# mit-acl/rl_collision_avoidance

Measured on AMD Instinct MI355X. Metric: agent-steps/sec (env.step) at 4 agents x 8192 worlds per GPU, higher is better.
Workload: dtype f64

## Files before the change

### __graft_entry__.py

```python
import os
import sys

ROOT = os.path.dirname(os.path.abspath(__file__))
if ROOT not in sys.path:
    sys.path.insert(0, ROOT)


def build() -> None:
    from rl_collision_avoidance_amd import build as hip_build
    path = hip_build.build(verbose=True)
    assert os.path.exists(path)
    try:
        for kind in (1, 2, 3, 4):
            hip_build.build_ulp_fault(kind)
    except Exception as exc:
        print("warning: development variant not built (%s); the tests that need it build it themselves" % exc)
    try:
        hip_build.build_crowd_dev()
    except Exception as exc:
        print("warning: crowd development variant not built (%s); tests/test_gpu_crowd.py builds it itself" % exc)
    from oracle import c_oracle
    c_oracle.build()
    import rl_collision_avoidance_amd
    from rl_collision_avoidance_amd import _lib
    handle = _lib.lib()
    for name, _, _ in _lib.SYMBOLS:
        getattr(handle, name)
    print("build ok:", path)


def smoke() -> None:
    import numpy as np
    import torch
    from oracle import c_oracle as co
    from rl_collision_avoidance_amd.batched_env import BatchedCollisionAvoidanceEnv

    assert torch.cuda.is_available(), "smoke() needs cuda:0"
    W, N, seed = 256, 4, 17
    env = BatchedCollisionAvoidanceEnv(W, device="cuda:0", seed=seed)
    env.reset()
    ocfg, ogen = co.default_cfg(N), co.default_gen(N, N, pool_size=int(env.cfg.gen_pool_size))
    st = co.State.empty(W, N)
    ep = np.zeros(W, np.uint32)
    co.generate(ocfg, ogen, seed, st, ep)
    rng = np.random.default_rng(seed)
    for t in range(40):
        acts = rng.integers(0, 11, size=(W, N)).astype(np.int32)
        obs, rew, done, go = env.step_autoreset(torch.from_numpy(acts).cuda())
        oobs, orew, odone, ogo = co.step_autoreset(ocfg, ogen, seed, st, ep, acts)
        assert np.array_equal(done.cpu().numpy(), odone) and np.array_equal(go.cpu().numpy(), ogo)
        d = np.abs(obs.cpu().numpy() - oobs)
        d[..., 3] = np.minimum(d[..., 3], np.abs(d[..., 3] - 2 * np.pi))
        assert d.max() <= 1e-5
        assert np.abs(rew.cpu().numpy() - orew).max() <= 1e-5
    fl = env.get_state()[2].cpu().numpy().view(np.uint32)
    assert np.array_equal(fl, st.flags)
    acts16 = rng.integers(0, 11, size=(16, W, N)).astype(np.int32)
    slots = env.new_step_slots(16, packed=True)
    pk_all, go_all = env.step_autoreset_packed(torch.from_numpy(acts16).cuda(), slots)
    wdt = env.obs_width
    for k in range(16):
        oobs, orew, odone, ogo = co.step_autoreset(ocfg, ogen, seed, st, ep, acts16[k])
        pk = pk_all[k].cpu().numpy()
        d = np.abs(pk[..., :wdt] - oobs)
        d[..., 3] = np.minimum(d[..., 3], np.abs(d[..., 3] - 2 * np.pi))
        assert d.max() <= 1e-5 and np.abs(pk[..., wdt] - orew).max() <= 1e-5, k
        assert np.array_equal(pk[..., wdt + 1].astype(np.uint8), odone) and np.array_equal(go_all[k].cpu().numpy(), ogo), k
    assert np.array_equal(env.get_state()[2].cpu().numpy().view(np.uint32), st.flags)
    obs = torch.from_numpy(np.ascontiguousarray(pk[..., :wdt])).cuda()
    from rl_collision_avoidance_amd.ga3c.network import NetworkVP_rnn
    from rl_collision_avoidance_amd.ga3c.policy_kernel import FusedPolicy
    net = NetworkVP_rnn(env.config).to("cuda:0")
    view = obs.view(W * N, -1)[:, 1:]
# ... 44 lines not shown
```

### rl_collision_avoidance_amd/build.py

```python
from __future__ import annotations

import os
import shutil
import subprocess

PKG_DIR = os.path.dirname(os.path.abspath(__file__))
ROOT = os.path.dirname(PKG_DIR)
CSRC = os.path.join(PKG_DIR, "csrc")
LIB_PATH = os.path.join(PKG_DIR, "libcavoid_hip.so")
SOURCES = [os.path.join(CSRC, "cavoid_capi.hip"), os.path.join(CSRC, "cavoid_multistep.hip"), os.path.join(CSRC, "cavoid_rvo.hip"),
           os.path.join(CSRC, "cavoid_relay.hip"), os.path.join(CSRC, "cavoid_quad.hip"), os.path.join(CSRC, "cavoid_rollout_capi.hip"),
           os.path.join(CSRC, "cavoid_policy_capi.hip"), os.path.join(CSRC, "cavoid_comm_capi.hip"), os.path.join(CSRC, "cavoid_actor.hip"),
           os.path.join(CSRC, "cavoid_actor_rvo.hip"), os.path.join(CSRC, "cavoid_actor_frozen.hip"), os.path.join(CSRC, "cavoid_crowd.hip"),
           os.path.join(CSRC, "cavoid_policy_ws.hip"), os.path.join(CSRC, "cavoid_policy_train_ring.hip"),
           os.path.join(CSRC, "cavoid_policy_wsring.hip"), os.path.join(CSRC, "cavoid_crowd_push.hip"), os.path.join(CSRC, "cavoid_crowd_rvo.hip"),
           os.path.join(CSRC, "cavoid_crowd_actor.hip")]
HEADERS = {
    "cavoid_capi.hip": ["cavoid_kernels.hpp", "cavoid_launch.hpp", "cavoid_host.hpp", "cavoid_crowd.hpp", "cavoid_crowd_rvo.hpp"],
    "cavoid_multistep.hip": ["cavoid_kernels.hpp", "cavoid_launch.hpp", "cavoid_host.hpp"],
    "cavoid_rvo.hip": ["cavoid_kernels.hpp", "cavoid_launch.hpp", "cavoid_host.hpp"],
    "cavoid_relay.hip": ["cavoid_kernels.hpp", "cavoid_relay.hpp", "cavoid_launch.hpp", "cavoid_host.hpp"],
    "cavoid_quad.hip": ["cavoid_kernels.hpp", "cavoid_quad.hpp", "cavoid_launch.hpp", "cavoid_host.hpp"],
    "cavoid_rollout_capi.hip": ["cavoid_rollout.hpp", "cavoid_rollout_host.hpp", "cavoid_host.hpp"],
    "cavoid_policy_capi.hip": ["cavoid_policy.hpp", "cavoid_policy_split.hpp", "cavoid_policy_split8.hpp", "cavoid_policy_crowd.hpp", "cavoid_policy_host.hpp",
# ... 116 lines not shown
    from concurrent.futures import ThreadPoolExecutor
    out = variant_path("ulp%d" % kind)
    if os.path.exists(out):
        return out
    build()
    objs = _compile_objects([], "", False, verbose)
    jobs, swap = [], {}
    for name in ("cavoid_capi.hip", "cavoid_multistep.hip", "cavoid_rvo.hip", "cavoid_relay.hip"):
        src = os.path.join(CSRC, name)
        obj = os.path.join(OBJ_DIR, name.replace(".hip", ".ulp%d.o" % kind))
        jobs.append([hipcc()] + FLAGS + EXTRA_FLAGS.get(name, []) + ["-DCAVOID_DEV_ULP_FAULT=%d" % kind, "-DCAVOID_DEV_ONLY_N", "-c", src, "-o", obj])
        swap[os.path.join(OBJ_DIR, name.replace(".hip", ".o"))] = obj
    if jobs:
        if verbose:
            for j in jobs:
                print(" ".join(j), flush=True)
        with ThreadPoolExecutor(max_workers=len(jobs)) as pool:
            list(pool.map(subprocess.check_call, jobs))
    for old in glob.glob(os.path.join(FAULT_DIR, "libcavoid_hip_ulp%d-*.so" % kind)):
        os.remove(old)
    tmp = out + ".tmp"
    _link([swap.get(o, o) for o in objs], tmp, verbose)
    os.replace(tmp, out)
    return out


def build_crowd_dev(verbose: bool = False) -> str:
    import glob
    from concurrent.futures import ThreadPoolExecutor
    out = variant_path("crowd2")
    if os.path.exists(out):
        return out
    build()
    objs = _compile_objects([], "", False, verbose)
    jobs, swap = [], {}
    for name in ("cavoid_capi.hip", "cavoid_multistep.hip", "cavoid_crowd.hip", "cavoid_crowd_rvo.hip"):
        src = os.path.join(CSRC, name)
        obj = os.path.join(OBJ_DIR, name.replace(".hip", ".crowd2.o"))
        jobs.append([hipcc()] + FLAGS + EXTRA_FLAGS.get(name, []) + ["-DCAVOID_DEV_CROWD_FROM_N=2", "-DCAVOID_DEV_ONLY_N", "-c", src, "-o", obj])
        swap[os.path.join(OBJ_DIR, name.replace(".hip", ".o"))] = obj
    if verbose:
        for j in jobs:
            print(" ".join(j), flush=True)
    with ThreadPoolExecutor(max_workers=len(jobs)) as pool:
        list(pool.map(subprocess.check_call, jobs))
    for old in glob.glob(os.path.join(FAULT_DIR, "libcavoid_hip_crowd2-*.so")):
        os.remove(old)
    tmp = out + ".tmp"
    _link([swap.get(o, o) for o in objs], tmp, verbose)
    os.replace(tmp, out)
    return out


if __name__ == "__main__":
    import sys
    if "--trace" in sys.argv:
        print(build_trace(verbose=True))
    elif "--crowd-dev" in sys.argv:
        print(build_crowd_dev(verbose=True))
    elif "--ulp-faults" in sys.argv:
        for kind in (1, 2, 3, 4):
            print(build_ulp_fault(kind, verbose=True))
    else:
        print(build(force=True, verbose=True))
```

### rl_collision_avoidance_amd/csrc/cavoid_kernels.hpp

```cpp
#pragma once
#include <hip/hip_runtime.h>
#include <stdint.h>

#include "cavoid.h"

namespace cavoid {

#ifdef CAVOID_TRACE
__device__ unsigned long long *g_trace = nullptr;
#define CAVOID_STAMP(k)                                                                \
    do {                                                                               \
        if (lane == 0 && g_trace) g_trace[wave * 16 + (k)] = (unsigned long long)clock64(); \
    } while (0)
#else
#define CAVOID_STAMP(k) do { } while (0)
#endif

#define CAVOID_RARE(x) __builtin_expect(!!(x), 0)
#ifndef CAVOID_SKIP
#define CAVOID_SKIP 0
#endif

constexpr double kPi = 3.14159265358979323846;
constexpr int kTileMaxAgents = 16;
// ... 255 lines not shown

__device__ __forceinline__ Ego ego_from(const KCfg &c, double tx, double ty, double heading) {
    Ego e;
    e.tx = tx;
    e.ty = ty;
    const double ss = e.tx * e.tx + e.ty * e.ty;
    const bool tiny = !(ss > 1e-16);
    double y = (double)__builtin_amdgcn_rsqf((float)ss);
    y = y * __builtin_fma(-0.5 * ss, y * y, 1.5);
    y = y * __builtin_fma(-0.5 * ss, y * y, 1.5);
    e.dist = tiny ? sqrt(ss) : ss * y;
    const double inv = tiny ? 1.0 : y;
    e.prll_x = e.tx * inv;
    e.prll_y = e.ty * inv;
    e.heading_ego = wrap_once(heading - (double)atan2f((float)e.ty, (float)e.tx), c.switches);
    return e;
}
__device__ __forceinline__ Ego ego_frame_obs(const KCfg &c, const Agent &a) { return ego_from(c, (double)a.gx - a.px, (double)a.gy - a.py, a.heading); }

__device__ __forceinline__ double time_to_impact(double rx, double ry, double vx, double vy, double R) {
    const double cc = rx * rx + ry * ry - R * R;
    if (cc <= 0.0) return 0.0;
    const double aa = vx * vx + vy * vy, bb = rx * vx + ry * vy;
    if (aa < 1e-10 || bb <= 0.0) return INFINITY;
    const double disc = bb * bb - aa * cc;
    if (disc < 0.0) return INFINITY;
    return (bb - sqrt(disc)) / aa;
}

__device__ __forceinline__ double sqrt_dist2(double x) {
    const double y = __builtin_amdgcn_rsq(fmax(x, 0x1p-1000));
    double g = x * y;
    double h = y * 0.5;
    const double r = __builtin_fma(-h, g, 0.5);
    g = __builtin_fma(g, r, g);
    h = __builtin_fma(h, r, h);
    double d = __builtin_fma(-g, g, x);
    g = __builtin_fma(d, h, g);
    d = __builtin_fma(-g, g, x);
    g = __builtin_fma(d, h, g);
    return g;
}

template <int N>
struct Others {
    static constexpr int K = N > 1 ? N - 1 : 1;
};

__device__ __forceinline__ int other_index(int i, int o, int n) {
    const int j = i + 1 + o;
    return j >= n ? j - n : j;
}

__device__ __forceinline__ uint32_t orderable(float f) {
    const uint32_t u = __float_as_uint(f + 0.0f);
    return u ^ ((u >> 31) ? 0xFFFFFFFFu : 0x80000000u);
}

struct Key {
    uint64_t v;
    __device__ __forceinline__ uint32_t hi() const { return (uint32_t)(v >> 32); }
    __device__ __forceinline__ uint32_t lo() const { return (uint32_t)v; }
    __device__ __forceinline__ void set(uint32_t hi, uint32_t lo) { v = ((uint64_t)hi << 32) | lo; }
};
constexpr uint32_t kKeyBias = 1u << 30;
constexpr uint32_t kKeySentinel = 0x7FFFFFF0u;
__device__ __forceinline__ bool key_is_sentinel(uint32_t hi) { return hi >= kKeySentinel; }
__device__ __forceinline__ int key_bucket(const Key &k) { return (int)(kKeyBias - k.hi()); }

struct OtherState { double px, py; float vxf, vyf, r; };

template <int N>
struct RingStage {
    static constexpr bool kDouble = N >= kRingDoubleFromN;
    const StageRec *self;
    const double *vx64, *vy64;
    int i, base;
    __device__ __forceinline__ OtherState other(int o) const {
        const StageRec *q = self + (o + 1);
        if (!kDouble) q = (o + 1 + i >= N) ? q - N : q;
        return OtherState{q->px, q->py, q->vxf, q->vyf, q->r};
    }
    __device__ __forceinline__ void vel64(int o, double &vx, double &vy) const {
        const int j = base + other_index(i, o, N);
        vx = vx64[j]; vy = vy64[j];
    }
};
template <int N>
struct ArrayStage {
    const double *px, *py, *vx, *vy;
    const float *r;
    int i, base;
    __device__ __forceinline__ OtherState other(int o) const {
        const int j = base + other_index(i, o, N);
        return OtherState{px[j], py[j], (float)vx[j], (float)vy[j], r[j]};
    }
    __device__ __forceinline__ void vel64(int o, double &ovx, double &ovy) const {
        const int j = base + other_index(i, o, N);
        ovx = vx[j]; ovy = vy[j];
    }
};

constexpr int kFeat = 5;
__device__ __forceinline__ void neighbour_features(const Ego &e, float pxf, float pyf, double rx, double ry, const OtherState &q, float (&f)[kFeat]) {
    f[0] = (float)__builtin_fma(rx, e.prll_x, ry * e.prll_y);
    f[1] = (float)__builtin_fma(ry, e.prll_x, -(rx * e.prll_y));
#if !defined(CAVOID_DEV_PKFORM)
    float t_par = q.vyf * pyf, t_orth = q.vxf * pyf;
    asm volatile("" : "+v"(t_par), "+v"(t_orth));
    f[2] = __builtin_fmaf(q.vxf, pxf, t_par);
    f[3] = __builtin_fmaf(q.vyf, pxf, -t_orth);
#else
    f[2] = __builtin_fmaf(q.vxf, pxf, q.vyf * pyf);
    f[3] = __builtin_fmaf(q.vyf, pxf, -(q.vxf * pyf));
#endif
    f[4] = q.r;
}

constexpr int kParkFromN = 6;
template <int N, bool PARK, bool SW, bool FEAT, class Stage>
__device__ __forceinline__ void pair_pass_impl(const KCfg &c, const Agent &a, const Ego &e, bool present, const Stage &st,
                                          Key (&key)[Others<N>::K], float (&gapf)[Others<N>::K], float (*feat)[kFeat],
                                          uint32_t &valid, bool &hit, double &min_gap, uint32_t *park, int lane, uint32_t frozen_w) {
    constexpr int K = Others<N>::K;
    const double ri = (double)a.radius;
    valid = 0u;
    hit = false;
    min_gap = INFINITY;
    if (!PARK) { key[0].set(kKeySentinel, 0u); gapf[0] = 0.0f; }
    auto one = [&](int o) {
        const OtherState q = st.other(o);
        const float rjf = q.r;
        const double rx = q.px - a.px, ry = q.py - a.py;
#if defined(CAVOID_DEV_ULP_FAULT) && CAVOID_DEV_ULP_FAULT == 1
        const double d = sqrt_dist2((double)((float)rx * (float)rx) + ry * ry);
#else
        const double d = sqrt_dist2(rx * rx + ry * ry);
#endif
        const bool other = present && (rjf >= 0.0f);
        bool collides = other;
        if (SW) {
            const int jj = other_index(st.i, o, N);
            collides = other && ((frozen_w >> jj) & 1u) == 0u && ((frozen_w >> st.i) & 1u) == 0u;
        }
        const double gap_c = d - (ri + (double)rjf);
        min_gap = collides ? fmin(min_gap, gap_c) : min_gap;
        hit = hit || (collides && gap_c <= c.collision_dist);
        const bool seen = other && !(d > c.horizon);
        valid |= seen ? (1u << o) : 0u;
        const double gap_o = d - ri - (double)rjf;
#if defined(CAVOID_DEV_ULP_FAULT) && CAVOID_DEV_ULP_FAULT == 3
        uint32_t hi = kKeyBias - (uint32_t)(int)rintf((float)gap_o * 100.0f);
#else
        uint32_t hi = kKeyBias - (uint32_t)(int)rint(gap_o * 100.0);
#endif
        uint32_t lo = orderable((float)(ry * e.tx - rx * e.ty));
        if (SW) {
            if (c.switches & kSwIndexTie) lo = (uint32_t)other_index(st.i, o, N);
            if (c.switches & kSwExactGap) { lo = 0u; hi = 0x7FFFFFFEu - (orderable((float)gap_o) >> 1); }
        }
        hi = seen ? hi : kKeySentinel + (uint32_t)o;
        if (PARK) {
            reinterpret_cast<uint64_t *>(park)[o * 64 + lane] = ((uint64_t)hi << 32) | lo;
            park[(2 * K + o) * 64 + lane] = __float_as_uint((float)gap_o);
        } else {
            gapf[o] = (float)gap_o;
            key[o].set(hi, lo);
        }
        if (FEAT) neighbour_features(e, (float)e.prll_x, (float)e.prll_y, rx, ry, q, feat[o]);
    };
    if (PARK) {
#pragma unroll 3
        for (int o = 0; o < N - 1; ++o) { one(o); __builtin_amdgcn_sched_barrier(0); }
    } else {
#pragma unroll
        for (int o = 0; o < N - 1; ++o) if (!(CAVOID_SKIP & 16) || o == 0) one(o);
    }
}

template <int N, bool PARK, bool FEAT, class Stage>
__device__ __forceinline__ void pair_pass(const KCfg &c, const Agent &a, const Ego &e, bool present, const Stage &st,
                                          Key (&key)[Others<N>::K], float (&gapf)[Others<N>::K], float (*feat)[kFeat],
                                          uint32_t &valid, bool &hit, double &min_gap, uint32_t *park = nullptr, int lane = 0,
                                          uint32_t frozen_w = 0u) {
    if (CAVOID_RARE(c.switches != 0u))
        pair_pass_impl<N, PARK, true, FEAT>(c, a, e, present, st, key, gapf, feat, valid, hit, min_gap, park, lane, frozen_w);
    else
        pair_pass_impl<N, PARK, false, FEAT>(c, a, e, present, st, key, gapf, feat, valid, hit, min_gap, park, lane, 0u);
}

#ifndef CAVOID_NT_STORES
// ... 1126 lines not shown
```

### rl_collision_avoidance_amd/csrc/cavoid_launch.hpp

```cpp
#pragma once
#include <hip/hip_runtime.h>
#include <hip/hip_ext.h>

#include <type_traits>

#include "cavoid.h"
#include "cavoid_host.hpp"
#include "cavoid_kernels.hpp"

struct cavoid_env {
    int device = 0;
    int64_t W = 0, A = 0, world_offset = 0;
    cavoid_cfg cfg{};
    cavoid::KCfg k{};
    cavoid::KState st{};
    cavoid::PoolRec *pool = nullptr;
    uint32_t *pool_episode = nullptr;
    int64_t pool_size = 0;
    int ahead_R = 0;
    uint32_t *ahead_hi[2] = {nullptr, nullptr};
    int ahead_cur = 0;
    int ahead_budget = 0;
    bool ahead_primed = false;
    bool ahead_always = false;
    int64_t ahead_refills = 0;
    int relay_topup_nc = -1;
    size_t relay_topup_lds = 0;
    bool relay_topup_fits = false;
    void *slab = nullptr;
    void *pool_slab = nullptr;
    double *d_actions = nullptr;
    int waves_per_block = 4;
    int grid = 0;
    int pipeline = 2;
    int relay_consumers = 3;
    int latency_mode = 0;
    int quad = -1;
    int prefetch_single = 0;
    int last_form = CAVOID_FORM_NONE;
    int last_relay_consumers = 0;
    hipEvent_t ev0 = nullptr, ev1 = nullptr;
};


namespace cavoid {

template <int... Ns>
struct NList {};
#ifdef CAVOID_DEV_ONLY_N
using EnvNs = NList<4, 10>;
using RelayNs = NList<4>;
using QuadNs = NList<4>;
#else
using EnvNs = NList<1, 2, 3, 4, 5, 6, 7, 8, 9, 10, 11, 12, 13, 14, 15, 16>;
using RelayNs = NList<1, 2, 3, 4, 5, 6>;
using QuadNs = NList<2, 3, 4, 5, 6, 10>;
#endif

#ifdef CAVOID_DEV_CROWD_FROM_N
constexpr int kCrowdFromN = CAVOID_DEV_CROWD_FROM_N;
#else
constexpr int kCrowdFromN = kTileMaxAgents + 1;
#endif
static inline bool crowd_form(int max_agents) { return max_agents >= kCrowdFromN; }

template <int... Ns, class F>
static inline int dispatch_n(int n, NList<Ns...>, F &&f) {
    int rc = CAVOID_EUNSUPPORTED;
    (void)((n == Ns ? (rc = f(std::integral_constant<int, Ns>{}), true) : false) || ...);
    return rc;
}

template <class K, class... Args>
static inline void launch_kernel(K kernel, dim3 grid, dim3 block, size_t lds, hipStream_t s, hipEvent_t ev_start, hipEvent_t ev_stop,
                                 const Args &...args) {
    if (ev_start || ev_stop) hipExtLaunchKernelGGL(kernel, grid, block, lds, s, ev_start, ev_stop, 0, args...);
    else hipLaunchKernelGGL(kernel, grid, block, lds, s, args...);
}

#ifdef CAVOID_TRACE
static inline int set_trace(unsigned long long *dev_ptr) {
    HIP_TRY(hipMemcpyToSymbol(HIP_SYMBOL(g_trace), &dev_ptr, sizeof(dev_ptr)));
    return CAVOID_OK;
}
#endif

static inline int note_form(cavoid_env *e, int rc, int form, int relay_consumers = 0) {
    if (rc == CAVOID_OK) {
        e->last_form = form;
        e->last_relay_consumers = relay_consumers;
    }
    return rc;
}

template <int MODE, bool RVO = false>
static inline int launch_on(cavoid_env *e, const KCfg &k, const KState &st, int grid_x, const KIO &io, hipStream_t s,
                     hipEvent_t ev_start, hipEvent_t ev_stop) {
    const dim3 grid(grid_x), block(64 * e->waves_per_block);
    const int row = io.obs ? io.obs_stride : k.width;
    int tile = (k.tile_rows * row + 3) & ~3;
    if (tile < k.park_floats) tile = k.park_floats;
    const size_t lds = (size_t)(lds_floats_block() + e->waves_per_block * (lds_floats_fixed(e->cfg.max_agents) + k.rvo_lds_floats + tile)) * sizeof(float);
    const int rc = dispatch_n(e->cfg.max_agents, EnvNs{}, [&](auto n) -> int {
        launch_kernel(env_kernel<decltype(n)::value, MODE, RVO>, grid, block, lds, s, ev_start, ev_stop, k, st, e->pool, io);
// ... 57 lines not shown
```

### rl_collision_avoidance_amd/csrc/cavoid_relay.hpp

```cpp
#pragma once
#include <cstddef>
#include <type_traits>

#include "cavoid_kernels.hpp"

namespace cavoid {

constexpr int kRelayMaxAgents = 6;
template <int N>
__host__ __device__ constexpr int relay_ring() { return N <= 5 ? 8 : 4; }
constexpr size_t kRelayLdsLimit = 80 * 1024;
constexpr int kRelayActRing = 64;
constexpr int kRelayActAhead = 48;
constexpr int kRelayEvq = 8;
constexpr int kRelayTopupMaxN = 5;

struct RelaySeq {
    int spec;
    int stage;
    int res;
    int fin;
    int act;
    int ev;
    int nxt;
// ... 217 lines not shown
template <int N, bool SW>
__device__ __forceinline__ void relay_pair_part(const KCfg &c, const Agent &a, const Ego &e, const bool present, const ArrayStage<N> &st, const int pw,
                                                const int lane, RelayCoop<N> &co, float (&gapf)[Others<N>::K], float (&feat)[Others<N>::K][kFeat]) {
    const double ri = (double)a.radius;
#pragma unroll
    for (int o = 0; o < N - 1; ++o) {
        if (o % kRelayCoopWaves != pw) continue;
        const OtherState q = st.other(o);
        const float rjf = q.r;
        const double rx = q.px - a.px, ry = q.py - a.py;
#if defined(CAVOID_DEV_ULP_FAULT) && CAVOID_DEV_ULP_FAULT == 1
        const double d = sqrt_dist2((double)((float)rx * (float)rx) + ry * ry);
#else
        const double d = sqrt_dist2(rx * rx + ry * ry);
#endif
        const bool other = present && (rjf >= 0.0f);
        const bool seen = other && !(d > c.horizon);
        const double gap_o = d - ri - (double)rjf;
#if defined(CAVOID_DEV_ULP_FAULT) && CAVOID_DEV_ULP_FAULT == 3
        uint32_t hi = kKeyBias - (uint32_t)(int)rintf((float)gap_o * 100.0f);
#else
        uint32_t hi = kKeyBias - (uint32_t)(int)rint(gap_o * 100.0);
#endif
        uint32_t lo = orderable((float)(ry * e.tx - rx * e.ty));
        if (SW) {
            if (c.switches & kSwIndexTie) lo = (uint32_t)other_index(st.i, o, N);
            if (c.switches & kSwExactGap) { lo = 0u; hi = 0x7FFFFFFEu - (orderable((float)gap_o) >> 1); }
        }
        hi = seen ? hi : kKeySentinel + (uint32_t)o;
        co.key[o][lane] = ((uint64_t)hi << 32) | lo;
        co.bits[o][lane] = seen ? 2u : 0u;
        gapf[o] = (float)gap_o;
        neighbour_features(e, (float)e.prll_x, (float)e.prll_y, rx, ry, q, feat[o]);
    }
}

struct RelayArgs { KCfg c; KState s; const PoolRec *pool; KIO io; };
static_assert(alignof(KCfg) == 8 && alignof(KState) == 8 && alignof(KIO) == 8 && alignof(RelayArgs) == 8, "kernel arguments: 8-byte aligned");
static_assert(sizeof(KCfg) % 8 == 0 && sizeof(KState) % 8 == 0 && sizeof(KIO) % 8 == 0, "kernel arguments: whole 8-byte words, no tail padding to skip");
static_assert(offsetof(RelayArgs, c) == 0 && offsetof(RelayArgs, s) == sizeof(KCfg) && offsetof(RelayArgs, pool) == sizeof(KCfg) + sizeof(KState) &&
                  offsetof(RelayArgs, io) == sizeof(KCfg) + sizeof(KState) + sizeof(const PoolRec *) &&
                  sizeof(RelayArgs) == sizeof(KCfg) + sizeof(KState) + sizeof(const PoolRec *) + sizeof(KIO),
              "RelayArgs must be the kernel's argument segment, argument by argument");
static_assert(sizeof(KIO) == 104 && offsetof(KIO, n_steps) == 80 && offsetof(KIO, ahead_hi) == 96, "KIO changed: check what relay_coop_last reads from it");
template <class T>
__device__ __forceinline__ void relay_load_args(T &dst, const __attribute__((address_space(4))) T *src) {
    static_assert(sizeof(T) % 4 == 0, "whole words");
    const __attribute__((address_space(4))) uint32_t *w = (const __attribute__((address_space(4))) uint32_t *)src;
    uint32_t d[sizeof(T) / 4];
#pragma unroll
    for (int k = 0; k < (int)(sizeof(T) / 4); ++k) d[k] = w[k];
    __builtin_memcpy(&dst, d, sizeof(T));
}
template <int N>
__device__ __forceinline__ void relay_coop_last(unsigned char *smem) {
    unsigned char *sp = smem + lds_floats_block() * sizeof(float);
    RelaySeq *seq = reinterpret_cast<RelaySeq *>(sp); sp += sizeof(RelaySeq) + kRelayEvq * sizeof(unsigned long long);
    const unsigned long long kp = (unsigned long long)(uint32_t)relay_peek(&seq->kernarg[0]) | ((unsigned long long)(uint32_t)relay_peek(&seq->kernarg[1]) << 32);
    typedef const __attribute__((address_space(4))) RelayArgs *ArgP;
    const ArgP ka = (ArgP)kp;
    KCfg c;
    KIO io;
    relay_load_args(c, &ka->c);
    relay_load_args(io, &ka->io);
    RelayTent *tents = reinterpret_cast<RelayTent *>(sp); sp += relay_ring<N>() * sizeof(RelayTent) + sizeof(RelayNxt);
    RelayRes *ress = reinterpret_cast<RelayRes *>(sp); sp += relay_ring<N>() * sizeof(RelayRes) + kRelayActRing * 64;
    RelayCoop<N> *coopb = reinterpret_cast<RelayCoop<N> *>(sp); sp += relay_coop_bytes<N>();
    float *tiles = reinterpret_cast<float *>(sp);
    const int lane0 = threadIdx.x & 63;
    const int tile_nc = relay_peek(&seq->tile_id);
    const int NC = tile_nc >> 16;
    const int role = relay_role_of(threadIdx.x >> 6, NC);
    const int pw = role < 2 ? role : 2;
    const int ostride = io.obs_stride;
    const int tile_floats = (c.tile_rows * ostride + 3) & ~3;
    const int wpw = c.wpw, lanes_used = wpw * N;
    const int64_t wave = tile_nc & 0xFFFF;
    const int64_t w0 = wave * wpw;
    const int lw = lane0 / N, i0 = lane0 - lw * N;
    const int64_t w = w0 + lw;
    const bool active = lane0 < lanes_used && w < c.num_worlds;
    const int base0 = lane0 < lanes_used ? lw * N : 0;
    const int64_t a_idx0 = w * N + i0;
    const bool packed = io.packed != 0;
    int64_t worlds_here = c.num_worlds - w0;
    if (worlds_here > wpw) worlds_here = wpw;
    if (worlds_here < 0) worlds_here = 0;
    const int n_steps = io.n_steps;
    constexpr int K = Others<N>::K;
    const int t = n_steps - 1;
    const int cid_l = t % NC;
    float *tile = tiles + (size_t)cid_l * tile_floats;
    RelayCoop<N> &co = *coopb;
    relay_wait_bounded(&seq->fin, t + 1);
    const RelayTent &f = tents[t & (relay_ring<N>() - 1)];
    const RelayRes &v = ress[t & (relay_ring<N>() - 1)];
    Agent ao;
    ao.px = f.px[lane0]; ao.py = f.py[lane0]; ao.vx = f.vx[lane0]; ao.vy = f.vy[lane0];
    ao.heading = f.heading[lane0]; ao.t_rem = 0.0;
    ao.gx = f.gx[lane0]; ao.gy = f.gy[lane0]; ao.speed = 0.0f;
    ao.radius = f.r[lane0]; ao.pref = f.pref[lane0]; ao.flags = v.flags[lane0];
    const uint32_t ctl_c = v.ctl[lane0];
    const float rew_c = v.rew[lane0], done_c = (ctl_c & 1u) ? 1.0f : 0.0f;
    const bool present = active && (ao.flags & CAVOID_F_PRESENT);
    const Ego e = ego_frame_obs(c, ao);
    const ArrayStage<N> as{f.px, f.py, f.vx, f.vy, f.r, i0, base0};
// ... 29 lines not shown
    }
    relay_coop_arrive(&seq->coop[1], lane0);
    if (io.out_step_stride == 0)
        for (int o = 0; o < NC; ++o) relay_wait_bounded(&seq->cfin[o], 1);
    const int64_t slot_w = (int64_t)t * io.out_step_stride;
    if (worlds_here > 0) {
        float *dst = io.obs + (slot_w + w0) * N * ostride;
        const bool lines = ((rows_active * ostride) & 31) == 0 && (reinterpret_cast<uintptr_t>(dst) & 127) == 0;
        if (io.out_step_stride != 0 && lines) flush_tile<4, true, true>(tile, dst, rows_active * ostride, pw * 64 + lane0, 64 * kRelayCoopWaves);
        else if (io.out_step_stride != 0) flush_tile<4, true>(tile, dst, rows_active * ostride, pw * 64 + lane0, 64 * kRelayCoopWaves);
        else flush_tile<4>(tile, dst, rows_active * ostride, pw * 64 + lane0, 64 * kRelayCoopWaves);
    }
    if (pw == 0 && active) {
        if (!packed) {
            io.rew[slot_w * N + a_idx0] = rew_c;
            io.done[slot_w * N + a_idx0] = (ctl_c & 1u) ? 1 : 0;
        }
        if (i0 == 0) io.game_over[slot_w + w] = (ctl_c & 2u) ? 1 : 0;
    }
    if (pw == 0) RELAY_MARK(29);
}

template <int N>
__device__ __forceinline__ void relay_topup() {
    __builtin_amdgcn_s_setprio(CAVOID_RELAY_PRIO_T);
    unsigned long long kp = (unsigned long long)__builtin_amdgcn_kernarg_segment_ptr();
    asm volatile("" : "+s"(kp));
    typedef const __attribute__((address_space(4))) RelayArgs *ArgP;
    const ArgP ka = (ArgP)kp;
    KCfg c;
    uint32_t *episode, *hi;
    const PoolRec *ring;
    relay_load_args(c, &ka->c);
    relay_load_args(episode, &ka->s.episode);
    relay_load_args(ring, &ka->pool);
    relay_load_args(hi, &ka->io.ahead_hi);
    const int lane0 = threadIdx.x & 63;
    const int wpw = c.wpw, lanes_used = wpw * N;
    const int lw = lane0 / N, i0 = lane0 - lw * N;
    const int64_t w = (int64_t)blockIdx.x * wpw + lw;
    const bool active = lane0 < lanes_used && w < c.num_worlds;
    const int base0 = lane0 < lanes_used ? lw * N : 0;
    uint32_t ep = 0u, fh = 0u;
    if (active) {
        ep = episode[w];
        fh = hi[w];
    }
    asm volatile("" : "+v"(ep), "+v"(fh));
    __syncthreads();
    ahead_fill_range<N, true>(c, ep, fh, active, w, i0, base0, lane0, hi, const_cast<PoolRec *>(ring), c.ahead, 0, 1, nullptr, nullptr);
}

template <int N>
__global__ void __launch_bounds__(64 * (4 + kRelayMaxConsumers), N <= kRelayTopupMaxN ? 4 : 1) env_relay_kernel(const KCfg c, const KState s, const PoolRec *pool, const KIO io) {
    extern __shared__ __attribute__((aligned(16))) unsigned char smem[];
    unsigned char *sp = smem;
    double *lds_tab = reinterpret_cast<double *>(sp); sp += lds_floats_block() * sizeof(float);
    RelaySeq *seq = reinterpret_cast<RelaySeq *>(sp); sp += sizeof(RelaySeq);
    unsigned long long *evq = reinterpret_cast<unsigned long long *>(sp); sp += kRelayEvq * sizeof(unsigned long long);
    RelayTent *tents = reinterpret_cast<RelayTent *>(sp); sp += relay_ring<N>() * sizeof(RelayTent);
    RelayNxt *nbuf = reinterpret_cast<RelayNxt *>(sp); sp += sizeof(RelayNxt);
    RelayRes *ress = reinterpret_cast<RelayRes *>(sp); sp += relay_ring<N>() * sizeof(RelayRes);
    unsigned char *actring = sp; sp += kRelayActRing * 64;
    RelayCoop<N> *coopb = reinterpret_cast<RelayCoop<N> *>(sp); sp += relay_coop_bytes<N>();
    float *tiles = reinterpret_cast<float *>(sp);

    const int NC = (blockDim.x >> 6) - 3 - (io.ahead_hi ? 1 : 0);
    const int role = relay_role_of(threadIdx.x >> 6, NC);
    const int lane0 = threadIdx.x & 63;
    const int ostride = io.obs_stride;
    const int tile_floats = (c.tile_rows * ostride + 3) & ~3;
    const int wpw = c.wpw, lanes_used = wpw * N;
    const int64_t wave = blockIdx.x;
    const int64_t w0 = wave * wpw;
    const int lw = lane0 / N, i0 = lane0 - lw * N;
    const int64_t w = w0 + lw;
    const bool active = lane0 < lanes_used && w < c.num_worlds;
    const int base0 = lane0 < lanes_used ? lw * N : 0;
    const int64_t a_idx0 = w * N + i0;
    const bool packed = io.packed != 0;
    int64_t worlds_here = c.num_worlds - w0;
    if (worlds_here > wpw) worlds_here = wpw;
    if (worlds_here < 0) worlds_here = 0;
    const int n_steps = io.n_steps;
    constexpr bool kCoop = N >= kRelayCoopFromN;
    const bool coop_role = role < 2 || role == 2 + NC;

    if (role == 0 && lane0 < (int)(sizeof(RelaySeq) / sizeof(int))) reinterpret_cast<int *>(seq)[lane0] = 0;
    if constexpr (kCoop) {
        if (role == 0 && lane0 == 0) {
            const unsigned long long kp = (unsigned long long)__builtin_amdgcn_kernarg_segment_ptr();
            seq->kernarg[0] = (int)(uint32_t)kp; seq->kernarg[1] = (int)(uint32_t)(kp >> 32);
            seq->tile_id = (int)blockIdx.x | (NC << 16);
        }
    }

    if (role == 0) {
        __builtin_amdgcn_s_setprio(CAVOID_RELAY_PRIO_D);
        RELAY_MARK(20);
        KCfg cd = c;
        asm volatile("" : "+s"(cd.dt), "+s"(cd.near_goal_sq), "+s"(cd.actions_fp32), "+s"(cd.dynamics),
                     "+s"(cd.timeout_enabled), "+s"(cd.switches));
        const RelayTrig trig = relay_trig_constants();
        Agent a;
        a.px = a.py = a.heading = a.t_rem = a.vx = a.vy = 0.0;
        a.gx = a.gy = a.radius = a.pref = a.speed = 0.0f;
        a.flags = 0u;
        uint32_t episode = 0u;
        double tab_v = 0.0;
        if (lane0 < 2 * c.num_actions) tab_v = c.action_table[lane0];
        int act0 = 0;
        if (active) {
            episode = s.episode[w];
            load_agent(s, a_idx0, a);
            act0 = io.actions[a_idx0];
        }
        if (cd.actions_fp32 && (lane0 & 1)) tab_v = (double)(float)tab_v;
        lds_tab[lane0] = tab_v;
        act0 = act0 < 0 ? 0 : (act0 >= c.num_actions ? c.num_actions - 1 : act0);
        const bool present_first = active && (a.flags & CAVOID_F_PRESENT);
        bool restarted_any = false, moved_any = false;
        int events = 0;
        bool T_moving;
        Agent T;
        wave_lds_sync();
        RelayStatics ks = relay_statics(a, active);
        T = relay_advance(cd, trig, a, ks, lds_tab[2 * act0], lds_tab[2 * act0 + 1], active, T_moving);
        __syncthreads();
        RELAY_MARK(21);
        double tab_s = 0.0, tab_h = 0.0;
        int act_q = 0;
        if (n_steps > 1) {
            const int actn = (int)actring[64 + lane0];
            tab_s = lds_tab[2 * actn]; tab_h = lds_tab[2 * actn + 1];
            if (n_steps > 2) act_q = (int)actring[2 * 64 + lane0];
        }
        auto stage_out = [&](RelayTent &tn, const Agent &x, float r_staged, int lane) {
            tn.px[lane] = x.px; tn.py[lane] = x.py; tn.r[lane] = r_staged; tn.flags[lane] = x.flags;
            tn.vx[lane] = x.vx; tn.vy[lane] = x.vy; tn.heading[lane] = x.heading;
            tn.gx[lane] = x.gx; tn.gy[lane] = x.gy; tn.pref[lane] = x.pref;
        };
        stage_out(tents[0], T, ks.r_staged, lane0);
        relay_post(&seq->spec, 1);
        relay_post(&seq->stage, 1);
        RELAY_MARK(22);
        int cslot = 0;
        for (int t = 0; t + 1 < n_steps; ++t) {
            int lane = lane0;
            asm volatile("" : "+v"(lane));
            RELAY_STAMP(0);
            RelayTent &tn = tents[(t + 1) & (relay_ring<N>() - 1)];
// ... 45 lines not shown
                        res->flags[lane] = nx.flags;
                    }
                }
                const bool s_present = active && (S.flags & CAVOID_F_PRESENT);
                const bool s_done = (S.flags & CAVOID_F_DONE_MASK) != 0u;
                const bool frozen = s_present && s_done && !restart;
                uint32_t fflags = S.flags;
                if (S.flags & CAVOID_F_AT_GOAL) fflags |= CAVOID_F_WAS_AT_GOAL;
                if (S.flags & CAVOID_F_IN_COLL) fflags |= CAVOID_F_WAS_IN_COLL;
                Tn.px = frozen ? S.px : Tn.px; Tn.py = frozen ? S.py : Tn.py; Tn.heading = frozen ? S.heading : Tn.heading;
                Tn.t_rem = frozen ? S.t_rem : Tn.t_rem;
                Tn.vx = frozen ? 0.0 : Tn.vx; Tn.vy = frozen ? 0.0 : Tn.vy; Tn.speed = frozen ? 0.0f : Tn.speed;
                Tn.flags = frozen ? fflags : Tn.flags;
                mn = frozen ? false : mn;
                stage_out(tn, Tn, ks.r_staged, lane);
                relay_post(&seq->stage, t + 2);
                if (rmask != 0ull) {
                    relay_wait(&seq->nxt, events + 1 - (kRelayEvq - 1));
                    if (lane == 0) evq[events & (kRelayEvq - 1)] = rmask;
                    events += 1;
                    relay_post(&seq->ev, events);
                }
            }
            T = Tn;
            T_moving = mn;
            tab_s = tab_s2; tab_h = tab_h2;
            act_q = act3;
            relay_post(&seq->fin, t + 1);
            RELAY_STAMP(3);
        }
        Agent S = T;
        {
            const int t = n_steps - 1;
            relay_spin(&seq->res, 2 * (t + 1));
            RelayRes *res = &ress[t & (relay_ring<N>() - 1)];
            const uint32_t vflags = res->flags[lane0], ctl = res->ctl[lane0];
            moved_any = moved_any || T_moving;
            S.flags = vflags;
            const bool restart = (ctl & 2u) != 0u;
            if (__ballot(restart) != 0ull) {
                relay_wait(&seq->nxt, events + 1);
                Agent nx;
                relay_read_nxt(*nbuf, lane0, nx);
                if (restart) {
                    S = nx; episode += 1u; restarted_any = true;
                    stage_out(tents[t & (relay_ring<N>() - 1)], nx, relay_statics(nx, active).r_staged, lane0);
                    res->flags[lane0] = nx.flags;
                }
            }
            relay_post(&seq->fin, t + 1);
        }
        RELAY_MARK(23);
        relay_post(&seq->stage, n_steps + 1);
        if (restarted_any) {
            store_agent(s, a_idx0, S);
            if (i0 == 0) s.episode[w] = episode;
        } else if (present_first) {
            if (moved_any) {
                s.px[a_idx0] = S.px; s.py[a_idx0] = S.py; s.heading[a_idx0] = S.heading; s.t_rem[a_idx0] = S.t_rem;
            }
            s.speed[a_idx0] = S.speed;
            s.flags[a_idx0] = S.flags;
        }
        RELAY_MARK(24);
    } else if (role == 1) {
        __builtin_amdgcn_s_setprio(CAVOID_RELAY_PRIO_P);
        KCfg cp = c;
        asm volatile("" : "+s"(cp.r_step), "+s"(cp.r_goal), "+s"(cp.r_coll), "+s"(cp.r_close), "+s"(cp.close_slope), "+s"(cp.close_range),
                     "+s"(cp.clip_lo), "+s"(cp.clip_hi), "+s"(cp.collision_dist), "+s"(cp.horizon), "+s"(cp.evaluate_mode));
        bool prev_surprise = false;
        __syncthreads();
        for (int t = 0; t < n_steps; ++t) {
            int lane = lane0, i = i0, base = base0;
            asm volatile("" : "+v"(lane), "+v"(i), "+v"(base));
            RELAY_STAMP(8);
            if (prev_surprise) relay_spin(&seq->stage, t + 1);
            else relay_spin(&seq->spec, t + 1);
            RELAY_STAMP(9);
            const RelayTent *tent = &tents[t & (relay_ring<N>() - 1)];
            Agent a;
            a.px = tent->px[lane]; a.py = tent->py[lane];
            a.radius = tent->r[lane];
            uint32_t flags = tent->flags[lane];
            const uint32_t flags_t = flags;
            const bool present = active && (flags & CAVOID_F_PRESENT);
            constexpr int K = Others<N>::K;
            bool hit = false;
            double min_gap = INFINITY;
            const double ri = (double)a.radius;
            RELAY_STAMP(12);
#pragma unroll
            for (int o = 0; o < ((CAVOID_RELAY_ABL & 2) ? 0 : N - 1); ++o) {
                const int j = base + other_index(i, o, N);
                const float rjf = tent->r[j];
                const double rx = tent->px[j] - a.px, ry = tent->py[j] - a.py;
                const double d = sqrt_dist2(rx * rx + ry * ry);
                const bool other = present && (rjf >= 0.0f);
                const double gap_c = d - (ri + (double)rjf);
                min_gap = other ? fmin(min_gap, gap_c) : min_gap;
                hit = hit || (other && gap_c <= cp.collision_dist);
            }
            RELAY_STAMP(13);
            const bool at_goal = (flags & CAVOID_F_AT_GOAL) != 0u;
            const bool may_collide = present && !at_goal && (flags & CAVOID_F_WAS_IN_COLL) == 0u;
            const bool collides = may_collide && hit;
            const bool close = may_collide && !hit && min_gap <= cp.close_range;
            double r = present ? cp.r_step : 0.0;
            r = (present && at_goal && (flags & CAVOID_F_WAS_AT_GOAL) == 0u) ? cp.r_goal : r;
            r = collides ? cp.r_coll : r;
            const double r_near = cp.r_close + cp.close_slope * min_gap;
            r = close ? r_near : r;
            flags |= collides ? CAVOID_F_IN_COLL : 0u;
            const double r_clip = fmin(fmax(r, cp.clip_lo), cp.clip_hi);
            r = present ? r_clip : r;
            const bool done = present ? (flags & CAVOID_F_DONE_MASK) != 0u : true;
            const unsigned long long running = __ballot(present && ((flags & CAVOID_F_LEARNING) || cp.evaluate_mode) && !done);
            const unsigned long long wmask = ((1ull << N) - 1ull) << base;
            const bool game_over = (running & wmask) == 0ull;
            const bool restart = active && game_over;
            const float rew_f = (float)r;
            RelayRes *res = &ress[t & (relay_ring<N>() - 1)];
            res->flags[lane] = flags;
            res->ctl[lane] = (done ? 1u : 0u) | (restart ? 2u : 0u);
            res->rew[lane] = rew_f;
            const bool new_coll = (flags & CAVOID_F_IN_COLL) != 0u && (flags_t & CAVOID_F_IN_COLL) == 0u;
            prev_surprise = !(CAVOID_RELAY_ABL & 24) && __ballot(new_coll || restart) != 0ull;
            relay_post(&seq->res, 2 * (t + 1) + (prev_surprise ? 1 : 0));
            RELAY_STAMP(10);
        }
    } else if (role == 2 + NC) {
        __builtin_amdgcn_s_setprio(CAVOID_RELAY_PRIO_L);
        RELAY_MARK(25);
        uint32_t ep = 0u;
        if (active) ep = s.episode[w];
        int loaded = 0;
        const int64_t a_safe = active ? a_idx0 : 0;
        auto load_actions = [&](int upto) {
            while (loaded < upto) {
                int v[8];
#pragma unroll
                for (int q = 0; q < 8; ++q) {
                    const int sidx = loaded + q < upto ? loaded + q : upto - 1;
                    v[q] = io.actions[(int64_t)sidx * io.action_stride + a_safe];
                }
#pragma unroll
                for (int q = 0; q < 8; ++q) {
                    int x = v[q] < 0 ? 0 : (v[q] >= c.num_actions ? c.num_actions - 1 : v[q]);
                    if (loaded + q < upto) actring[((loaded + q) & (kRelayActRing - 1)) * 64 + lane0] = (unsigned char)x;
                }
                loaded = loaded + 8 < upto ? loaded + 8 : upto;
            }
        };
        load_actions(n_steps < 8 ? n_steps : 8);
        RELAY_MARK(26);
        __syncthreads();
        relay_post(&seq->act, loaded);
        {
            Agent r0;
            absent_agent(r0);
            if (active) load_pool(pool, (int64_t)pool_index(c, (uint32_t)(c.world_offset + w), ep + 1u) * N + i0, r0);
            RelayNxt &nb = *nbuf;
            nb.px[lane0] = r0.px; nb.py[lane0] = r0.py; nb.heading[lane0] = r0.heading; nb.t_rem[lane0] = r0.t_rem;
            nb.gx[lane0] = r0.gx; nb.gy[lane0] = r0.gy; nb.radius[lane0] = r0.radius; nb.pref[lane0] = r0.pref;
            nb.flags[lane0] = r0.flags;
            relay_post(&seq->nxt, 1);
            RELAY_MARK(27);
        }
        int served = 0, idle_polls = 0;
        while (true) {
            const int ev = relay_peek(&seq->ev), fin = relay_peek(&seq->fin);
            if (served < ev) {
                asm volatile("" ::: "memory");
                const unsigned long long mask = evq[served & (kRelayEvq - 1)];
                if ((mask >> lane0) & 1ull) {
                    ep += 1u;
                    Agent r0;
                    load_pool(pool, (int64_t)pool_index(c, (uint32_t)(c.world_offset + w), ep + 1u) * N + i0, r0);
                    RelayNxt &nb = *nbuf;
                    nb.px[lane0] = r0.px; nb.py[lane0] = r0.py; nb.heading[lane0] = r0.heading; nb.t_rem[lane0] = r0.t_rem;
                    nb.gx[lane0] = r0.gx; nb.gy[lane0] = r0.gy; nb.radius[lane0] = r0.radius; nb.pref[lane0] = r0.pref;
                    nb.flags[lane0] = r0.flags;
                }
                served += 1;
                idle_polls = 0;
                relay_post(&seq->nxt, served + 1);
                continue;
            }
            if (loaded < n_steps && loaded < fin + kRelayActAhead) {
                int upto = fin + kRelayActAhead;
                if (upto > loaded + 8) upto = loaded + 8;
                if (upto > n_steps) upto = n_steps;
                load_actions(upto);
                idle_polls = 0;
                relay_post(&seq->act, loaded);
                continue;
            }
            if (fin >= n_steps && relay_peek(&seq->stage) > n_steps) break;
            if (++idle_polls > kRelayPollLimit) __builtin_trap();
            __builtin_amdgcn_s_sleep(2);
        }
    } else if (role == 3 + NC) {
        relay_topup<N>();
    } else {
        __builtin_amdgcn_s_setprio(CAVOID_RELAY_PRIO_C);
        KCfg cc = c;
        asm volatile("" : "+s"(cc.switches));
        const int cid = role - 2;
        float *tile = tiles + (size_t)cid * tile_floats;
        __syncthreads();
        const int n_mine = kCoop ? n_steps - 1 : n_steps;
        for (int t = cid; t < n_mine; t += NC) {
            int lane = lane0, i = i0, base = base0;
            asm volatile("" : "+v"(lane), "+v"(i), "+v"(base));
            RELAY_STAMP(16);
            relay_wait_bounded(&seq->fin, t + 1);
            RELAY_STAMP(17);
            if (CAVOID_RELAY_ABL & 1) { relay_post(&seq->cons[cid], t + 1); continue; }
            const RelayTent &f = tents[t & (relay_ring<N>() - 1)];
            const RelayRes &v = ress[t & (relay_ring<N>() - 1)];
            Agent ao;
            ao.px = f.px[lane]; ao.py = f.py[lane]; ao.vx = f.vx[lane]; ao.vy = f.vy[lane];
            ao.heading = f.heading[lane]; ao.t_rem = 0.0;
            ao.gx = f.gx[lane]; ao.gy = f.gy[lane]; ao.speed = 0.0f;
            ao.radius = f.r[lane]; ao.pref = f.pref[lane]; ao.flags = v.flags[lane];
            const uint32_t ctl_c = v.ctl[lane];
            const float rew_c = v.rew[lane], done_c = (ctl_c & 1u) ? 1.0f : 0.0f;
            const bool present = active && (ao.flags & CAVOID_F_PRESENT);
            const Ego e = ego_frame_obs(cc, ao);
            Key key[Others<N>::K];
            float gapf[Others<N>::K];
            uint32_t valid;
            bool hit;
            double min_gap;
            const ArrayStage<N> as{f.px, f.py, f.vx, f.vy, f.r, i, base};
            float feat[Others<N>::K][kFeat];
            pair_pass<N, false, true>(cc, ao, e, present, as, key, gapf, feat, valid, hit, min_gap);
            RELAY_STAMP(18);
            const bool last = t == n_steps - 1 && io.out_step_stride == 0;
            const int64_t slot_w = (int64_t)t * io.out_step_stride;
            auto order_last = [&]() {
                if (last)
                    for (int o = 0; o < NC; ++o)
                        if (o != cid) relay_wait_bounded(&seq->cfin[o], 1);
            };
            assemble_obs<N, false, true, ArrayStage<N>, decltype(order_last)>(cc, ao, e, active, lane, as, key, gapf, feat, valid, tile,
                                         io.obs + (slot_w + w0) * N * ostride, (int)worlds_here * N, ostride, packed, rew_c, done_c, wave,
                                         order_last, io.out_step_stride != 0);
            if (active) {
                if (!packed) {
                    io.rew[slot_w * N + a_idx0] = rew_c;
                    io.done[slot_w * N + a_idx0] = (ctl_c & 1u) ? 1 : 0;
                }
                if (i0 == 0) io.game_over[slot_w + w] = (ctl_c & 2u) ? 1 : 0;
            }
            relay_post(&seq->cons[cid], t + 1);
            RELAY_STAMP(19);
            if (t == 0) RELAY_MARK(28);
// ... 15 lines not shown
```

Measured before the change: 24.11 billion.

## Share symmetric pairwise distances across mirror lanes and reload kernel args per role

Pairwise distances are symmetric, so each lane now computes only about half of its N-1 pair distances and fetches the rest from the partner lane. For N=4 the fetch is a DPP quad permute; other N use a shuffle. The relay kernel also loads its arguments per role from the kernarg segment and pins them in scalar registers, aiming to lower register pressure. A plain-distance build variant is added for testing; the risk is extra cross-lane latency and possible rounding differences.

Result: faster. 25.02 billion, median of 6 (+3.8%).

```diff
diff --git a/__graft_entry__.py b/__graft_entry__.py
--- a/__graft_entry__.py
+++ b/__graft_entry__.py
@@ -19,6 +19,10 @@
         hip_build.build_crowd_dev()
     except Exception as exc:
         print("warning: crowd development variant not built (%s); tests/test_gpu_crowd.py builds it itself" % exc)
+    try:
+        hip_build.build_plain_dist()
+    except Exception as exc:
+        print("warning: plain-distance development variant not built (%s); tests/test_gpu_relay_trim.py builds it itself" % exc)
     from oracle import c_oracle
     c_oracle.build()
     import rl_collision_avoidance_amd
diff --git a/rl_collision_avoidance_amd/build.py b/rl_collision_avoidance_amd/build.py
--- a/rl_collision_avoidance_amd/build.py
+++ b/rl_collision_avoidance_amd/build.py
@@ -192,10 +192,41 @@
     return out
 
 
+def build_plain_dist(verbose: bool = False) -> str:
+    import glob
+    from concurrent.futures import ThreadPoolExecutor
+    out = variant_path("plaindist")
+    if os.path.exists(out):
+        return out
+    build()
+    objs = _compile_objects([], "", False, verbose)
+    jobs, swap = [], {}
+    for name in ("cavoid_capi.hip", "cavoid_multistep.hip", "cavoid_rvo.hip", "cavoid_relay.hip"):
+        src = os.path.join(CSRC, name)
+        obj = os.path.join(OBJ_DIR, name.replace(".hip", ".plaindist.o"))
+        jobs.append([hipcc()] + FLAGS + EXTRA_FLAGS.get(name, []) +
+                    ["-DCAVOID_MIRROR_DIST=0", "-DCAVOID_RELAY_ROLE_ARGS=0", "-DCAVOID_DEV_ONLY_N", "-DCAVOID_DEV_ENV_NS=3,4,5,6,10",
+                     "-DCAVOID_DEV_RELAY_NS=3,4,5,6", "-c", src, "-o", obj])
+        swap[os.path.join(OBJ_DIR, name.replace(".hip", ".o"))] = obj
+    if verbose:
+        for j in jobs:
+            print(" ".join(j), flush=True)
+    with ThreadPoolExecutor(max_workers=len(jobs)) as pool:
+        list(pool.map(subprocess.check_call, jobs))
+    for old in glob.glob(os.path.join(FAULT_DIR, "libcavoid_hip_plaindist-*.so")):
+        os.remove(old)
+    tmp = out + ".tmp"
+    _link([swap.get(o, o) for o in objs], tmp, verbose)
+    os.replace(tmp, out)
+    return out
+
+
 if __name__ == "__main__":
     import sys
     if "--trace" in sys.argv:
         print(build_trace(verbose=True))
+    elif "--plain-dist" in sys.argv:
+        print(build_plain_dist(verbose=True))
     elif "--crowd-dev" in sys.argv:
         print(build_crowd_dev(verbose=True))
     elif "--ulp-faults" in sys.argv:
diff --git a/rl_collision_avoidance_amd/csrc/cavoid_kernels.hpp b/rl_collision_avoidance_amd/csrc/cavoid_kernels.hpp
--- a/rl_collision_avoidance_amd/csrc/cavoid_kernels.hpp
+++ b/rl_collision_avoidance_amd/csrc/cavoid_kernels.hpp
@@ -331,6 +331,37 @@
     return j >= n ? j - n : j;
 }
 
+#ifndef CAVOID_MIRROR_DIST
+#define CAVOID_MIRROR_DIST 1
+#endif
+template <int N>
+__host__ __device__ constexpr int mirror_computed() { return (CAVOID_MIRROR_DIST && N >= 3) ? N / 2 : (N > 1 ? N - 1 : 1); }
+__host__ __device__ constexpr int other_index_c(int i, int o, int n) { return i + 1 + o >= n ? i + 1 + o - n : i + 1 + o; }
+template <int N>
+__host__ __device__ constexpr bool mirror_split_ok() {
+    for (int i = 0; i < N; ++i)
+        for (int o = mirror_computed<N>(); o < N - 1; ++o)
+            if (N - 2 - o < 0 || N - 2 - o >= mirror_computed<N>() || other_index_c(other_index_c(i, o, N), N - 2 - o, N) != i) return false;
+    return true;
+}
+static_assert(mirror_split_ok<3>() && mirror_split_ok<4>() && mirror_split_ok<5>() && mirror_split_ok<6>() && mirror_split_ok<7>() && mirror_split_ok<8>() &&
+                  mirror_split_ok<9>() && mirror_split_ok<10>() && mirror_split_ok<11>() && mirror_split_ok<12>() && mirror_split_ok<13>() && mirror_split_ok<14>() &&
+                  mirror_split_ok<15>() && mirror_split_ok<16>(), "mirror_computed: a fetched slot must be one the mirror lane computes");
+#if CAVOID_MIRROR_DIST
+static_assert(mirror_computed<4>() == 2 && other_index_c(0, 2, 4) == ((0x93 >> 0) & 3) && other_index_c(1, 2, 4) == ((0x93 >> 2) & 3) &&
+                  other_index_c(2, 2, 4) == ((0x93 >> 4) & 3) && other_index_c(3, 2, 4) == ((0x93 >> 6) & 3),
+              "mirror_fetch<4>: quad_perm 0x93 must read lane other_index(i, 2, 4) of the quad");
+#endif
+template <int N>
+__device__ __forceinline__ double mirror_fetch(double mine, int src) {
+    if (N == 4) {
+        const int lo = __builtin_amdgcn_update_dpp(0, __double2loint(mine), 0x93, 0xF, 0xF, true);
+        const int hi = __builtin_amdgcn_update_dpp(0, __double2hiint(mine), 0x93, 0xF, 0xF, true);
+        return __hiloint2double(hi, lo);
+    }
+    return __shfl(mine, src);
+}
+
 __device__ __forceinline__ uint32_t orderable(float f) {
     const uint32_t u = __float_as_uint(f + 0.0f);
     return u ^ ((u >> 31) ? 0xFFFFFFFFu : 0x80000000u);
@@ -407,15 +438,24 @@
     hit = false;
     min_gap = INFINITY;
     if (!PARK) { key[0].set(kKeySentinel, 0u); gapf[0] = 0.0f; }
+    constexpr int kOwn = PARK ? K : mirror_computed<N>();
+    constexpr bool kMirror = kOwn < N - 1;
+    double dk[kMirror ? kOwn : 1];
     auto one = [&](int o) {
         const OtherState q = st.other(o);
         const float rjf = q.r;
         const double rx = q.px - a.px, ry = q.py - a.py;
+        double d;
+        if (!kMirror || o < kOwn) {
 #if defined(CAVOID_DEV_ULP_FAULT) && CAVOID_DEV_ULP_FAULT == 1
-        const double d = sqrt_dist2((double)((float)rx * (float)rx) + ry * ry);
+            d = sqrt_dist2((double)((float)rx * (float)rx) + ry * ry);
 #else
-        const double d = sqrt_dist2(rx * rx + ry * ry);
+            d = sqrt_dist2(rx * rx + ry * ry);
 #endif
+            if constexpr (kMirror) dk[o] = d;
+        } else {
+            d = mirror_fetch<N>(dk[N - 2 - o], st.base + other_index(st.i, o, N));
+        }
         const bool other = present && (rjf >= 0.0f);
         bool collides = other;
         if (SW) {
diff --git a/rl_collision_avoidance_amd/csrc/cavoid_launch.hpp b/rl_collision_avoidance_amd/csrc/cavoid_launch.hpp
--- a/rl_collision_avoidance_amd/csrc/cavoid_launch.hpp
+++ b/rl_collision_avoidance_amd/csrc/cavoid_launch.hpp
@@ -48,8 +48,14 @@
 template <int... Ns>
 struct NList {};
 #ifdef CAVOID_DEV_ONLY_N
-using EnvNs = NList<4, 10>;
-using RelayNs = NList<4>;
+#ifndef CAVOID_DEV_ENV_NS
+#define CAVOID_DEV_ENV_NS 4, 10
+#endif
+#ifndef CAVOID_DEV_RELAY_NS
+#define CAVOID_DEV_RELAY_NS 4
+#endif
+using EnvNs = NList<CAVOID_DEV_ENV_NS>;
+using RelayNs = NList<CAVOID_DEV_RELAY_NS>;
 using QuadNs = NList<4>;
 #else
 using EnvNs = NList<1, 2, 3, 4, 5, 6, 7, 8, 9, 10, 11, 12, 13, 14, 15, 16>;
diff --git a/rl_collision_avoidance_amd/csrc/cavoid_relay.hpp b/rl_collision_avoidance_amd/csrc/cavoid_relay.hpp
--- a/rl_collision_avoidance_amd/csrc/cavoid_relay.hpp
+++ b/rl_collision_avoidance_amd/csrc/cavoid_relay.hpp
@@ -293,6 +293,48 @@
     for (int k = 0; k < (int)(sizeof(T) / 4); ++k) d[k] = w[k];
     __builtin_memcpy(&dst, d, sizeof(T));
 }
+#ifndef CAVOID_RELAY_ROLE_ARGS
+#define CAVOID_RELAY_ROLE_ARGS 1
+#endif
+typedef const __attribute__((address_space(4))) RelayArgs *RelayArgP;
+#if CAVOID_RELAY_ROLE_ARGS
+#define RELAY_ROLE_ARGS_LOAD()                                                                         \
+    unsigned long long kp_ = (unsigned long long)__builtin_amdgcn_kernarg_segment_ptr();               \
+    asm volatile("" : "+s"(kp_));                                                                      \
+    KCfg c; KState s; const PoolRec *pool; KIO io;                                                     \
+    relay_load_args(s, &((RelayArgP)kp_)->s); relay_load_args(io, &((RelayArgP)kp_)->io);               \
+    relay_load_args(c, &((RelayArgP)kp_)->c); relay_load_args(pool, &((RelayArgP)kp_)->pool);            \
+    asm volatile("" : "+s"(c.wpw), "+s"(c.num_worlds))
+#define RELAY_ROLE_PIN(...) asm volatile("" : __VA_ARGS__)
+#define RELAY_ROLE_STATE(name)                                                                         \
+    unsigned long long kps_ = (unsigned long long)__builtin_amdgcn_kernarg_segment_ptr();              \
+    asm volatile("" : "+s"(kps_));                                                                     \
+    KState name;                                                                                       \
+    relay_load_args(name, &((RelayArgP)kps_)->s)
+#else
+#define RELAY_ROLE_ARGS_LOAD() const KCfg &c = c_; const KState &s = s_; const PoolRec *const pool = pool_; const KIO &io = io_
+#define RELAY_ROLE_STATE(name) const KState &name = s_
+#define RELAY_ROLE_PIN(...) do { } while (0)
+#endif
+#define RELAY_ROLE_ARGS()                                                                              \
+    RELAY_ROLE_ARGS_LOAD();                                                                            \
+    (void)s; (void)pool;                                                                               \
+    [[maybe_unused]] const int ostride = io.obs_stride;                                                \
+    [[maybe_unused]] const int tile_floats = (c.tile_rows * ostride + 3) & ~3;                         \
+    const int wpw = c.wpw, lanes_used = wpw * N;                                                       \
+    [[maybe_unused]] const int64_t wave = blockIdx.x;                      \
+    const int64_t w0 = wave * wpw;                                                                     \
+    const int lw = lane0 / N;                                                                          \
+    [[maybe_unused]] const int i0 = lane0 - lw * N;                                                    \
+    [[maybe_unused]] const int64_t w = w0 + lw;                                                        \
+    [[maybe_unused]] const bool active = lane0 < lanes_used && w < c.num_worlds;                       \
+    [[maybe_unused]] const int base0 = lane0 < lanes_used ? lw * N : 0;                                \
+    [[maybe_unused]] const int64_t a_idx0 = w * N + i0;                                                \
+    [[maybe_unused]] const bool packed = io.packed != 0;                                               \
+    [[maybe_unused]] int64_t worlds_here = c.num_worlds - w0;                                          \
+    if (worlds_here > wpw) worlds_here = wpw;                                                          \
+    if (worlds_here < 0) worlds_here = 0;                                                              \
+    [[maybe_unused]] const int n_steps = io.n_steps
 template <int N>
 __device__ __forceinline__ void relay_coop_last(unsigned char *smem) {
     unsigned char *sp = smem + lds_floats_block() * sizeof(float);
@@ -428,7 +470,7 @@
 }
 
 template <int N>
-__global__ void __launch_bounds__(64 * (4 + kRelayMaxConsumers), N <= kRelayTopupMaxN ? 4 : 1) env_relay_kernel(const KCfg c, const KState s, const PoolRec *pool, const KIO io) {
+__global__ void __launch_bounds__(64 * (4 + kRelayMaxConsumers), N <= kRelayTopupMaxN ? 4 : 1) env_relay_kernel(const KCfg c_, const KState s_, const PoolRec *pool_, const KIO io_) {
     extern __shared__ __attribute__((aligned(16))) unsigned char smem[];
     unsigned char *sp = smem;
     double *lds_tab = reinterpret_cast<double *>(sp); sp += lds_floats_block() * sizeof(float);
@@ -441,24 +483,9 @@
     RelayCoop<N> *coopb = reinterpret_cast<RelayCoop<N> *>(sp); sp += relay_coop_bytes<N>();
     float *tiles = reinterpret_cast<float *>(sp);
 
-    const int NC = (blockDim.x >> 6) - 3 - (io.ahead_hi ? 1 : 0);
+    const int NC = (blockDim.x >> 6) - 3 - (io_.ahead_hi ? 1 : 0);
     const int role = relay_role_of(threadIdx.x >> 6, NC);
     const int lane0 = threadIdx.x & 63;
-    const int ostride = io.obs_stride;
-    const int tile_floats = (c.tile_rows * ostride + 3) & ~3;
-    const int wpw = c.wpw, lanes_used = wpw * N;
-    const int64_t wave = blockIdx.x;
-    const int64_t w0 = wave * wpw;
-    const int lw = lane0 / N, i0 = lane0 - lw * N;
-    const int64_t w = w0 + lw;
-    const bool active = lane0 < lanes_used && w < c.num_worlds;
-    const int base0 = lane0 < lanes_used ? lw * N : 0;
-    const int64_t a_idx0 = w * N + i0;
-    const bool packed = io.packed != 0;
-    int64_t worlds_here = c.num_worlds - w0;
-    if (worlds_here > wpw) worlds_here = wpw;
-    if (worlds_here < 0) worlds_here = 0;
-    const int n_steps = io.n_steps;
     constexpr bool kCoop = N >= kRelayCoopFromN;
     const bool coop_role = role < 2 || role == 2 + NC;
 
@@ -473,6 +500,9 @@
 
     if (role == 0) {
         __builtin_amdgcn_s_setprio(CAVOID_RELAY_PRIO_D);
+        RELAY_ROLE_ARGS();
+        RELAY_ROLE_PIN("+s"(s.px), "+s"(s.py), "+s"(s.heading), "+s"(s.t_rem), "+s"(s.gx), "+s"(s.gy), "+s"(s.radius), "+s"(s.pref), "+s"(s.flags),
+                       "+s"(s.episode), "+s"(io.actions), "+s"(c.action_table));
         RELAY_MARK(20);
         KCfg cd = c;
         asm volatile("" : "+s"(cd.dt), "+s"(cd.near_goal_sq), "+s"(cd.actions_fp32), "+s"(cd.dynamics),
@@ -624,19 +654,21 @@
         }
         RELAY_MARK(23);
         relay_post(&seq->stage, n_steps + 1);
+        RELAY_ROLE_STATE(sw);
         if (restarted_any) {
-            store_agent(s, a_idx0, S);
-            if (i0 == 0) s.episode[w] = episode;
+            store_agent(sw, a_idx0, S);
+            if (i0 == 0) sw.episode[w] = episode;
         } else if (present_first) {
             if (moved_any) {
-                s.px[a_idx0] = S.px; s.py[a_idx0] = S.py; s.heading[a_idx0] = S.heading; s.t_rem[a_idx0] = S.t_rem;
-            }
-            s.speed[a_idx0] = S.speed;
-            s.flags[a_idx0] = S.flags;
+                sw.px[a_idx0] = S.px; sw.py[a_idx0] = S.py; sw.heading[a_idx0] = S.heading; sw.t_rem[a_idx0] = S.t_rem;
+            }
+            sw.speed[a_idx0] = S.speed;
+            sw.flags[a_idx0] = S.flags;
         }
         RELAY_MARK(24);
     } else if (role == 1) {
         __builtin_amdgcn_s_setprio(CAVOID_RELAY_PRIO_P);
+        RELAY_ROLE_ARGS();
         KCfg cp = c;
         asm volatile("" : "+s"(cp.r_step), "+s"(cp.r_goal), "+s"(cp.r_coll), "+s"(cp.r_close), "+s"(cp.close_slope), "+s"(cp.close_range),
                      "+s"(cp.clip_lo), "+s"(cp.clip_hi), "+s"(cp.collision_dist), "+s"(cp.horizon), "+s"(cp.evaluate_mode));
@@ -661,12 +693,21 @@
             double min_gap = INFINITY;
             const double ri = (double)a.radius;
             RELAY_STAMP(12);
+            constexpr int kOwn = mirror_computed<N>();
+            constexpr bool kMirror = kOwn < N - 1;
+            double dk[kMirror ? kOwn : 1];
 #pragma unroll
             for (int o = 0; o < ((CAVOID_RELAY_ABL & 2) ? 0 : N - 1); ++o) {
                 const int j = base + other_index(i, o, N);
                 const float rjf = tent->r[j];
-                const double rx = tent->px[j] - a.px, ry = tent->py[j] - a.py;
-                const double d = sqrt_dist2(rx * rx + ry * ry);
+                double d;
+                if (!kMirror || o < kOwn) {
+                    const double rx = tent->px[j] - a.px, ry = tent->py[j] - a.py;
+                    d = sqrt_dist2(rx * rx + ry * ry);
+                    if constexpr (kMirror) dk[o] = d;
+                } else {
+                    d = mirror_fetch<N>(dk[N - 2 - o], j);
+                }
                 const bool other = present && (rjf >= 0.0f);
                 const double gap_c = d - (ri + (double)rjf);
                 min_gap = other ? fmin(min_gap, gap_c) : min_gap;
@@ -702,6 +743,8 @@
         }
     } else if (role == 2 + NC) {
         __builtin_amdgcn_s_setprio(CAVOID_RELAY_PRIO_L);
+        RELAY_ROLE_ARGS();
+        RELAY_ROLE_PIN("+s"(s.episode), "+s"(io.actions), "+s"(io.action_stride), "+s"(c.num_actions));
         RELAY_MARK(25);
         uint32_t ep = 0u;
         if (active) ep = s.episode[w];
@@ -775,6 +818,7 @@
         relay_topup<N>();
     } else {
         __builtin_amdgcn_s_setprio(CAVOID_RELAY_PRIO_C);
+        RELAY_ROLE_ARGS();
         KCfg cc = c;
         asm volatile("" : "+s"(cc.switches));
         const int cid = role - 2;
```
